# facebookresearch/spdl

Measured on AMD Instinct MI355X. Metric: images/sec device-resident JPEG→RGB224, 1/2/4/8×MI355X; % HBM roofline, higher is better.
Workload: dtype u8; 1 GPU; configs[1]: synthetic 480x640 q90 4:2:0 baseline JPEG resident in HBM -> RGB 224x224 u8 (scale bicubic decrease + centred pad, rgb24); global_batch=256, per_gpu_batch=256, distinct_images=32, lanes=4, hw_queues=4, entropy_threads=256, entropy_piece_bytes=131072

## Files before the change

spdl_amd/csrc/hj_common.h:

```cpp
#pragma once
#include <stddef.h>
#include <stdint.h>

#ifndef HJ_HD
#define HJ_HD __host__ __device__
#endif

namespace hj {

constexpr int kMaxComp = 4;

enum { kColorGray = 0, kColorYcbcr, kColorRgb, kColorCmyk, kColorYcck, kColorYcbcrk };
inline HJ_HD bool frame_color(int ncomp, const int32_t* h, const int32_t* v, const int* ids,
                              int adobe, int32_t* color) {
  bool all11 = true;
  for (int c = 0; c < ncomp; c++) all11 = all11 && h[c] == 1 && v[c] == 1;
  if (ncomp == 1) {
    *color = kColorGray;
  } else if (ncomp == 3) {
    const bool rgb = adobe == 0 || (ids[0] == 'R' && ids[1] == 'G' && ids[2] == 'B');
    if (rgb && !all11) return false;
    *color = rgb ? kColorRgb : kColorYcbcr;
  } else {
    if (!all11) return false;
// ... 69 lines not shown
  int32_t sub_lo;
  int32_t maxcode[18];
  int32_t valoff[17];
  uint8_t vals[256];
};

enum { kSwsX = 0, kSwsOne = 1, kSwsTwo = 2 };
enum SwsTable { kHlPos = 0, kHlCoef, kHcPos, kHcCoef, kVlPos, kVlCoef, kVcPos, kVcCoef, kVmode, kSwsTables };
struct SwsDesc {
  int32_t sw, sh;
  int32_t chr_w;
  int32_t full, gray;
  int32_t hl_taps, hc_taps, vl_taps, vc_taps;
  int32_t hl_size, hc_size, vl_size, vc_size;
  int32_t off[kSwsTables];
  int32_t rb;
  int32_t col_chunk;
  int32_t gbr;
  int32_t pre, pre_rl, pre_rc;
  int32_t yuv, hsub, vsub, chr_h;
};

struct ImageDesc {
  int64_t in_off;
  int64_t in_size;
  int64_t coef_off;
  int64_t plane_off[kMaxComp];
  int64_t seg_off;
  int64_t out_off;
  int64_t wt_off;
  int32_t seg_cap;
  int32_t width, height, ncomp;
  int32_t h_samp[kMaxComp], v_samp[kMaxComp];
  int32_t nblocks;
  int32_t plane_stride[kMaxComp];
  int32_t dx, dy, ow, oh;
  SwsDesc sws;
  int64_t ds_off;
  int32_t ds_cap;
  int32_t color;
  int64_t rec_off;
  int64_t rec_cap;
  int32_t pieces;
  int32_t chain_off;
  int32_t ds_wg0, idct_wg0;
  int32_t hs_wg0, hs_wgs;
  int32_t sws_wg0, sws_bands, sws_chunks;
  int64_t hbuf_off;
  int32_t refuse;
  int32_t pad_;
};

#ifndef HJ_SWS_LDS_KB
#define HJ_SWS_LDS_KB 32
#endif
constexpr int kSwsLdsBudget = HJ_SWS_LDS_KB * 1024;
constexpr int kSwsMaxCols = 256;
inline HJ_HD int sws_col_stride(int rows) { return 2 * (((rows + 5) >> 1) | 1); }

struct ImageInfo {
  int32_t status;
  int32_t width, height, ncomp, hmax, vmax, mcux, mcuy, bpm, nblocks, ri;
  int32_t scan_start;
  int32_t comp_h[kMaxComp], comp_v[kMaxComp];
  int32_t comp_bw[kMaxComp], comp_bh[kMaxComp];
  int32_t comp_w[kMaxComp], comp_hpx[kMaxComp];
  int32_t mcu_comp[kMaxBpm], mcu_dx[kMaxBpm], mcu_dy[kMaxBpm];
  int32_t dc_tab[kMaxComp], ac_tab[kMaxComp];
  uint16_t qt[kMaxComp][64];
  int32_t nseg;
  int32_t clean_len;
  int32_t sync_rounds;
  int32_t scan_end;
  int32_t ent_wide;
  int32_t multiscan;
  int32_t progressive;
  int32_t color;
  int32_t tab_off[8], tab_n[8];
  uint32_t tab_hash[8];
  int32_t lut_ref[8];
  int64_t tphase[4];
  int64_t dbg[4];
  int32_t sdiag[48];
};

constexpr int kDsChunk = 4096;
#ifndef HJ_IDCT_THREADS
#define HJ_IDCT_THREADS 256
#endif
constexpr int kIdctThreads = HJ_IDCT_THREADS;
constexpr int kHsRows = 16;
struct DsChunk {
  int32_t keep, rst, term;
  int32_t keep_pre, rst_pre;
  int32_t pad_[3];
};

struct SwsCsc {
  int32_t crv, cbu, cgu, cgv;
  int32_t y_coeff, y_offset, v2r, v2g, u2g, u2b;
};

#ifndef HJ_ABLATIONS
#define HJ_ABLATIONS 0
#endif
enum Ablate : int32_t {
  kAblSwsHpass = 0x100,
  kAblSwsVpass = 0x200,
  kAblSwsStore = 0x400,
  kAblIdctNone = 0x800,
  kAblEntWrite = 0x1000,
  kAblEntSync = 0x2000,
  kAblEntList = 0x4000,
  kAblEntDc = 0x8000,
  kAblEntDesc = 0x80000,
  kAblEntropy = kAblEntWrite | kAblEntSync | kAblEntList | kAblEntDc | kAblEntDesc,
  kAblNoMultiscan = 0x10000,
  kAblNoIdct = 0x20000,
  kAblNoOutput = 0x40000,
};

struct BatchParams {
  int32_t n;
  int32_t pix_fmt, dtype, idct;
  int32_t resize, filter;
  int32_t out_w, out_h;
  int32_t sub_bits;
  int32_t debug_mask;
  int32_t xcd_order;
  float mean[3], std[3];
  SwsCsc csc;
};
static_assert(sizeof(BatchParams) == 108 && offsetof(BatchParams, csc) == 68, "BatchParams layout");

struct EntropyParams {
  int32_t sub_bits;
  int32_t warm_slots;
  int32_t min_run_slots;
  int32_t chain_after;
  int32_t prio;
  int32_t ablate;
  int64_t handoff_ticks;
};

enum Status {
  kOk = 0,
  kErrNotJpeg = 1,
  kErrUnsupported = 2,
  kErrBadHeader = 3,
  kErrBadHuffman = 4,
  kErrTruncated = 5,
  kErrBadRestart = 6,
  kErrBadGeometry = 7,
  kErrDevice = 9,
  kErrHandoff = 11,
};

}
```

spdl_amd/csrc/hj_kernels.hip:

```cpp
#include <hip/hip_fp16.h>
#include <hip/hip_runtime.h>

#include "hj_common.h"
#include "hj_destuff.h"
#include "hj_idct.h"
#include "hj_launch.h"
#include "hj_sws_tile.h"

namespace hj {

__device__ __forceinline__ uint32_t rfl(uint32_t v) { return __builtin_amdgcn_readfirstlane(v); }


struct ParseScratch {
  ImageInfo info;
  uint16_t qt[4][64];
  uint8_t bits[8][17];
  uint8_t vals[8][256];
  int32_t have[8];
  int32_t qhave[4];
  int32_t maxcode[8][18];
  int32_t valoff[8][17];
  int32_t dqt_off[4], dqt_pq[4];
  int32_t dht_off[8], dht_n[8];
// ... 104 lines not shown
        if (in.comp_h[c] < 1 || in.comp_h[c] > 4 || in.comp_v[c] < 1 || in.comp_v[c] > 4 ||
            comp_tq[c] > 3)
          return kErrBadHeader;
      }
      if (!frame_color(nf, in.comp_h, in.comp_v, comp_id, adobe, &in.color)) return kErrUnsupported;
      have_sof = 1;
    } else if (m == 0xC3 || (m >= 0xC5 && m <= 0xC7) || (m >= 0xC9 && m <= 0xCB) ||
               (m >= 0xCD && m <= 0xCF)) {
      return kErrUnsupported;
    } else if (m == 0xEE) {
      if (n >= 12 && p[0] == 'A' && p[1] == 'd' && p[2] == 'o' && p[3] == 'b' && p[4] == 'e')
        adobe = p[11];
    } else if (m == 0xDD) {
      if (n < 2) return kErrBadHeader;
      in.ri = be16(p);
    } else if (m == 0xDA) {
      if (!have_sof) return kErrBadHeader;
      int ns = p[0];
      if (ns < 1 || ns > in.ncomp) return kErrBadHeader;
      in.multiscan = prog || ns != in.ncomp;
      in.progressive = prog;
      if (n < 1 + 2 * ns + 3) return kErrBadHeader;
      int32_t* order = s.order;
      for (int i = 0; i < kMaxComp; i++) order[i] = 0;
      for (int i = 0; i < ns; i++) {
        int cs = p[1 + 2 * i], c = -1;
        for (int k = 0; k < in.ncomp; k++)
          if (comp_id[k] == cs) c = k;
        if (c < 0) return kErrBadHeader;
        order[i] = c;
        in.dc_tab[c] = p[2 + 2 * i] >> 4;
        in.ac_tab[c] = p[2 + 2 * i] & 15;
        if (in.dc_tab[c] > 3 || in.ac_tab[c] > 3) return kErrBadHeader;
      }
      int ss = p[1 + 2 * ns], se = p[2 + 2 * ns], ahal = p[3 + 2 * ns];
      if (!in.multiscan && (ss != 0 || se != 63 || ahal != 0)) return kErrUnsupported;
      in.scan_start = pos;
      if (in.multiscan)
        for (int i = 0; i < in.ncomp; i++) order[i] = i;
      int hmax = 1, vmax = 1;
      for (int c = 0; c < in.ncomp; c++) {
        hmax = max(hmax, in.comp_h[c]);
        vmax = max(vmax, in.comp_v[c]);
      }
      in.hmax = hmax;
      in.vmax = vmax;
      for (int c = 0; c < in.ncomp; c++) {
        if (hmax % in.comp_h[c] || vmax % in.comp_v[c]) return kErrUnsupported;
        if (!s.qhave[comp_tq[c]] ||
            (!in.multiscan && (!s.have[in.dc_tab[c]] || !s.have[4 + in.ac_tab[c]])))
          return kErrBadHeader;
        in.comp_w[c] = (in.width * in.comp_h[c] + hmax - 1) / hmax;
        in.comp_hpx[c] = (in.height * in.comp_v[c] + vmax - 1) / vmax;
        s.qtsel[c] = comp_tq[c];
      }
      if (in.ncomp == 1) {
        in.comp_bw[0] = (in.comp_w[0] + 7) / 8;
        in.comp_bh[0] = (in.comp_hpx[0] + 7) / 8;
        in.mcux = in.comp_bw[0];
        in.mcuy = in.comp_bh[0];
        in.bpm = 1;
        in.mcu_comp[0] = 0;
        in.mcu_dx[0] = in.mcu_dy[0] = 0;
      } else {
        in.mcux = (in.width + 8 * hmax - 1) / (8 * hmax);
        in.mcuy = (in.height + 8 * vmax - 1) / (8 * vmax);
        int b = 0;
        for (int i = 0; i < (in.multiscan ? in.ncomp : ns); i++) {
          int c = order[i];
          in.comp_bw[c] = in.mcux * in.comp_h[c];
          in.comp_bh[c] = in.mcuy * in.comp_v[c];
          for (int y = 0; y < in.comp_v[c]; y++)
            for (int x = 0; x < in.comp_h[c]; x++) {
              if (b >= kMaxBpm) return kErrUnsupported;
              in.mcu_comp[b] = c;
              in.mcu_dx[b] = x;
              in.mcu_dy[b] = y;
              b++;
            }
        }
        in.bpm = b;
      }
      in.nblocks = in.mcux * in.mcuy * in.bpm;
      return kOk;
    }
  }
}

__global__ void __launch_bounds__(256, 8) parse_kernel(const uint8_t* __restrict__ bytes,
                                                    const ImageDesc* __restrict__ host_desc,
                                                    ImageDesc* __restrict__ desc,
                                                    ImageInfo* __restrict__ infos,
                                                    HuffTable* __restrict__ luts,
                                                    const uint4* __restrict__ host_tables,
                                                    uint4* __restrict__ tables, int64_t ntab16,
                                                    const uint32_t* __restrict__ host_work,
                                                    uint32_t* __restrict__ work, int nwork,
                                                    uint64_t* __restrict__ chain,
                                                    uint32_t* __restrict__ ds_map,
                                                    uint32_t* __restrict__ idct_map,
                                                    uint32_t* __restrict__ hs_map,
                                                    uint32_t* __restrict__ sws_map) {
  __shared__ ParseScratch s;
  __shared__ int st;
  __shared__ __attribute__((aligned(16))) uint8_t hdr[kHdrBytes];
  const int img = blockIdx.x, tid = threadIdx.x;
#if HJ_PARSE_PROF
  int64_t pt[8];
  int npt = 0;
  pt[npt++] = wall_clock64();
#define HJ_PT() (pt[npt++] = wall_clock64())
#else
#define HJ_PT() ((void)0)
#endif
  __shared__ __attribute__((aligned(16))) ImageDesc sdd;
  {
    static_assert(sizeof(ImageDesc) % 8 == 0, "descriptor copied in 8-byte words");
    const uint64_t* src = reinterpret_cast<const uint64_t*>((host_desc ? host_desc : desc) + img);
    uint64_t* dst = reinterpret_cast<uint64_t*>(desc + img);
    uint64_t* sdst = reinterpret_cast<uint64_t*>(&sdd);
    for (int i = tid; i < (int)(sizeof(ImageDesc) / 8); i += blockDim.x) {
      const uint64_t v = src[i];
      if (host_desc) dst[i] = v;
      sdst[i] = v;
    }
  }
  if (host_desc) {
    for (int64_t i = (int64_t)img * blockDim.x + tid; i < ntab16;
         i += (int64_t)gridDim.x * blockDim.x)
      tables[i] = host_tables[i];
    for (int i = img * blockDim.x + tid; i < nwork; i += gridDim.x * blockDim.x)
      work[i] = host_work[i];
  }
  __syncthreads();
  const ImageDesc& dd = sdd;
  for (int i = tid; i < dd.ds_cap; i += blockDim.x) ds_map[dd.ds_wg0 + i] = (uint32_t)img;
  for (int i = tid; i < (dd.nblocks + kIdctThreads - 1) / kIdctThreads; i += blockDim.x)
    idct_map[dd.idct_wg0 + i] = (uint32_t)img;
  for (int i = tid; i < dd.hs_wgs; i += blockDim.x) hs_map[dd.hs_wg0 + i] = (uint32_t)img;
  for (int i = tid; i < dd.sws_bands * dd.sws_chunks; i += blockDim.x)
    sws_map[dd.sws_wg0 + i] = (uint32_t)img;
  if (img == 0 && tid == 0) chain[0] = 0ull;
  if (dd.pieces > 1)
    for (int i = tid; i < dd.pieces * kChainGranules; i += blockDim.x)
      chain[kChainHead + dd.chain_off + i] = 0ull;
  {
    int* z = reinterpret_cast<int*>(&s);
    for (int i = tid; i < (int)(sizeof(ParseScratch) / 4); i += blockDim.x) z[i] = 0;
  }
  const int nh = (int)min(dd.in_size, (int64_t)kHdrBytes) & ~15;
  for (int i = tid; i < nh / 16; i += blockDim.x)
    reinterpret_cast<uint4*>(hdr)[i] = reinterpret_cast<const uint4*>(bytes + dd.in_off)[i];
  __syncthreads();
  HJ_PT();
  if (tid == 0) {
    const Bytes file{bytes + dd.in_off, (lds_u8*)hdr, nh};
    int rc = parse_headers(file, (int)dd.in_size, s);
    if (rc == kOk) {
      if (s.info.width != dd.width || s.info.height != dd.height || s.info.ncomp != dd.ncomp ||
          s.info.nblocks != dd.nblocks || s.info.color != dd.color)
        rc = kErrBadHeader;
      for (int c = 0; c < s.info.ncomp && rc == kOk; c++)
        if (s.info.comp_h[c] != dd.h_samp[c] || s.info.comp_v[c] != dd.v_samp[c])
          rc = kErrBadHeader;
      if (rc == kOk && s.info.ri > 0 &&
          (s.info.mcux * s.info.mcuy + s.info.ri - 1) / s.info.ri > dd.seg_cap)
// ... 3446 lines not shown
      {
        const int2 rn = wr ? ms_decode_refine<MsWBits>(S, si, soft, geo, in, d, cl, sizeu, lv,
                                                       masks, lane)
                           : ms_decode_refine<MsBits>(S, si, soft, geo, in, d, cl, sizeu, lv,
                                                      masks, lane);
        rc = ms_i(rn.x);
        nsym = ms_i(rn.y);
      }
#endif
#undef HJ_MS_SCAN
      ms_publish(S, si, 1 << 30);
      if (ms_lane0() && si < 16) {
        S.sdiag[3 * si] = (int32_t)(ts - tdec);
        S.sdiag[3 * si + 1] = (int32_t)(wall_clock64() - tdec);
        S.sdiag[3 * si + 2] = nsym;
#ifdef HJ_MS_PROF
        if (prof[1]) {
          S.sdiag[3 * si] = (int32_t)(prof[0] >> 8);
          S.sdiag[3 * si + 1] = (int32_t)(prof[1] >> 8);
          S.sdiag[3 * si + 2] = (int32_t)(prof[2] >> 8);
        }
#endif
      }
      if (ms_lane0()) {
        if (rc != kOk) atomicCAS(&S.err, kOk, rc);
        const int sss = ms_i(sc.ss), sah = ms_i(sc.ah);
        const int kind = !progu ? 3 : (sss == 0 ? 0 : (sah == 0 ? 1 : 2));
        atomicAdd(reinterpret_cast<unsigned long long*>(&S.tkind[kind]),
                  (unsigned long long)(wall_clock64() - ts));
        __hip_atomic_fetch_or(&S.done, 1ull << si, __ATOMIC_RELEASE, __HIP_MEMORY_SCOPE_WORKGROUP);
      }
    }
    __builtin_amdgcn_s_setprio(0);
  }
  __syncthreads();
  tph[2] = wall_clock64() - tdec;
#pragma unroll
  for (int i = 0; i < 4; i++) tdbg[i] = S.tkind[i];
  tdbg[3] = (int64_t)__builtin_amdgcn_s_memtime() - cdec;
  tph[1] = 0;
  if (S.err != kOk) {
    if (tid == 0) in.status = S.err;
    return;
  }
  for (int j = tid; j < nblocks; j += nt) {
    const int c = in.mcu_comp[j % in.bpm];
    uint4 q[16];
    const uint4* src = reinterpret_cast<const uint4*>(lv + (size_t)j * 64);
#pragma unroll
    for (int i = 0; i < 16; i++) q[i] = src[i];
    int32_t l[64];
#pragma unroll
    for (int i = 0; i < 16; i++) {
      l[4 * i] = (int32_t)q[i].x;
      l[4 * i + 1] = (int32_t)q[i].y;
      l[4 * i + 2] = (int32_t)q[i].z;
      l[4 * i + 3] = (int32_t)q[i].w;
    }
    uint32_t* out = ents + ((size_t)dd.coef_off + j) * 64;
    uint32_t n = 0;
#pragma unroll
    for (int k = 1; k < 64; k++) {
      if (l[k] != 0) {
        out[n++] = ((uint32_t)l[k] << 16) | (uint32_t)k;
      }
    }
    const int32_t dc = (int32_t)(int16_t)(uint16_t)((uint32_t)kDcBias + (uint32_t)l[0] * in.qt[c][0]);
    bdesc[(size_t)dd.coef_off + j] = make_uint2((uint32_t)j * 64u, n | ((uint32_t)dc << 16));
  }
  __syncthreads();
  if (tid == 0) {
    tph[3] = wall_clock64() - t0 - tph[0] - tph[1] - tph[2];
    for (int i = 0; i < 4; i++) in.tphase[i] = tph[i];
    for (int i = 0; i < 4; i++) in.dbg[i] = tdbg[i];
    for (int i = 0; i < 48; i++) in.sdiag[i] = S.sdiag[i];
    in.sync_rounds = S.nscans;
  }
}


constexpr int kBlkWords = 32;

typedef int16_t __attribute__((may_alias)) hj_i16_alias;

template <int NT>
__device__ __forceinline__ uint32_t slot_byte(uint32_t s) {
  return (s >> 1) * (uint32_t)NT * 4u + ((s & 1u) << 1);
}

template <int NT>
__device__ __forceinline__ void load_dequant(uint32_t (&sq)[kMaxComp][64], const ImageInfo& in,
                                             int tid) {
  for (int k = tid; k < kMaxComp * 64; k += NT)
    sq[k >> 6][k & 63] = slot_byte<NT>(kSlotOrder[k & 63]) | ((uint32_t)in.qt[k >> 6][k & 63] << 16);
}

template <int NT>
__device__ __forceinline__ void list_block(const uint32_t* __restrict__ ents, const uint2 bd,
                                           const int64_t coef_off, const int nblocks,
                                           const uint32_t* sqc, uint32_t* b32) {
#pragma unroll
  for (int w = 0; w < kBlkWords; w++) b32[w * NT] = w == 0 ? (bd.y >> 16) : 0u;
  uint8_t* blk = reinterpret_cast<uint8_t*>(b32);
  uint8_t* dummy = reinterpret_cast<uint8_t*>(b32 + kBlkWords * NT);
  const uint32_t cap = (uint32_t)nblocks * 64u;
  const uint32_t lo = bd.x & 3u, start = bd.x & ~3u;
  uint32_t count = min(bd.y & 0xFFFFu, 63u);
  if (start > cap - 64u) count = 0;
  const uint32_t hi_e = lo + count;
  const uint4* e4 = reinterpret_cast<const uint4*>(ents + (size_t)coef_off * 64 + start);
  const uint32_t n4 = (hi_e + 3u) >> 2;
  for (uint32_t i = 0; i < n4; i += 4) {
    uint4 q[4];
#pragma unroll
    for (int u = 0; u < 4; u++) q[u] = e4[min(i + u, n4 - 1u)];
#pragma unroll
    for (int u = 0; u < 4; u++) {
      const uint32_t w[4] = {q[u].x, q[u].y, q[u].z, q[u].w};
#pragma unroll
      for (int h = 0; h < 4; h++) {
        const uint32_t k = 4u * (i + u) + h;
        const uint32_t qs = sqc[w[h] & 63u];
        uint8_t* dst = k >= lo && k < hi_e ? blk + (qs & 0xFFFFu) : dummy;
        *reinterpret_cast<hj_i16_alias*>(dst) = (int16_t)pk_mul_lo16(w[h] >> 16, qs >> 16);
      }
    }
  }
}

typedef short hj_s16x2 __attribute__((ext_vector_type(2)));
__device__ __forceinline__ int32_t dot2(uint32_t a, uint32_t w, int32_t c) {
  return __builtin_amdgcn_sdot2(__builtin_bit_cast(hj_s16x2, a), __builtin_bit_cast(hj_s16x2, w),
                                c, false);
}
constexpr uint32_t pk16(int lo, int hi) {
  return (uint32_t)(uint16_t)(int16_t)lo | ((uint32_t)(uint16_t)(int16_t)hi << 16);
}
__device__ __forceinline__ uint32_t pack_lo16(uint32_t lo, uint32_t hi) {
  return __builtin_amdgcn_perm(hi, lo, 0x05040100u);
}
__device__ __forceinline__ void sidct8(uint32_t e0, uint32_t e1, uint32_t o0, uint32_t o1,
                                       int32_t bias, int32_t (&a)[4], int32_t (&b)[4]) {
  a[0] = dot2(e1, pk16(kW4, kW6), dot2(e0, pk16(kW4, kW2), bias));
  a[1] = dot2(e1, pk16(-kW4, -kW2), dot2(e0, pk16(kW4, kW6), bias));
  a[2] = dot2(e1, pk16(-kW4, kW2), dot2(e0, pk16(kW4, -kW6), bias));
  a[3] = dot2(e1, pk16(kW4, -kW6), dot2(e0, pk16(kW4, -kW2), bias));
  b[0] = dot2(o1, pk16(kW5, kW7), dot2(o0, pk16(kW1, kW3), 0));
  b[1] = dot2(o1, pk16(-kW1, -kW5), dot2(o0, pk16(kW3, -kW7), 0));
  b[2] = dot2(o1, pk16(kW7, kW3), dot2(o0, pk16(kW5, -kW1), 0));
  b[3] = dot2(o1, pk16(kW3, -kW1), dot2(o0, pk16(kW7, -kW5), 0));
}
template <int NT>
__device__ __forceinline__ uint4 blk_row(const uint32_t* b32, int i) {
  return make_uint4(b32[(4 * i) * NT], b32[(4 * i + 1) * NT], b32[(4 * i + 2) * NT],
                    b32[(4 * i + 3) * NT]);
}
template <int NT>
__device__ __forceinline__ void simple_idct_slots(const uint32_t* b32, int32_t (&px)[64]) {
  uint32_t r[8][8];
#pragma unroll
  for (int i = 0; i < 8; i++) {
    const uint4 q = blk_row<NT>(b32, i);
    int32_t a[4], b[4];
    sidct8(q.x, q.y, q.z, q.w, 1 << 10, a, b);
    const bool dc_only = ((q.x >> 16) | q.y | q.z | q.w) == 0u;
    const uint32_t dc = q.x << 3;
    r[i][0] = dc_only ? dc : (uint32_t)((int32_t)((uint32_t)a[0] + (uint32_t)b[0]) >> 11);
    r[i][7] = dc_only ? dc : (uint32_t)((int32_t)((uint32_t)a[0] - (uint32_t)b[0]) >> 11);
    r[i][1] = dc_only ? dc : (uint32_t)((int32_t)((uint32_t)a[1] + (uint32_t)b[1]) >> 11);
    r[i][6] = dc_only ? dc : (uint32_t)((int32_t)((uint32_t)a[1] - (uint32_t)b[1]) >> 11);
    r[i][2] = dc_only ? dc : (uint32_t)((int32_t)((uint32_t)a[2] + (uint32_t)b[2]) >> 11);
    r[i][5] = dc_only ? dc : (uint32_t)((int32_t)((uint32_t)a[2] - (uint32_t)b[2]) >> 11);
    r[i][3] = dc_only ? dc : (uint32_t)((int32_t)((uint32_t)a[3] + (uint32_t)b[3]) >> 11);
    r[i][4] = dc_only ? dc : (uint32_t)((int32_t)((uint32_t)a[3] - (uint32_t)b[3]) >> 11);
  }
#pragma unroll
  for (int k = 0; k < 8; k++) {
    int32_t a[4], b[4];
    sidct8(pack_lo16(r[0][k], r[2][k]), pack_lo16(r[4][k], r[6][k]), pack_lo16(r[1][k], r[3][k]),
           pack_lo16(r[5][k], r[7][k]), kW4 * ((1 << 19) / kW4), a, b);
    px[k] = clip_u8_opaque((int32_t)((uint32_t)a[0] + (uint32_t)b[0]) >> 20);
    px[8 + k] = clip_u8_opaque((int32_t)((uint32_t)a[1] + (uint32_t)b[1]) >> 20);
    px[16 + k] = clip_u8_opaque((int32_t)((uint32_t)a[2] + (uint32_t)b[2]) >> 20);
    px[24 + k] = clip_u8_opaque((int32_t)((uint32_t)a[3] + (uint32_t)b[3]) >> 20);
    px[32 + k] = clip_u8_opaque((int32_t)((uint32_t)a[3] - (uint32_t)b[3]) >> 20);
    px[40 + k] = clip_u8_opaque((int32_t)((uint32_t)a[2] - (uint32_t)b[2]) >> 20);
    px[48 + k] = clip_u8_opaque((int32_t)((uint32_t)a[1] - (uint32_t)b[1]) >> 20);
    px[56 + k] = clip_u8_opaque((int32_t)((uint32_t)a[0] - (uint32_t)b[0]) >> 20);
  }
}

template <int NT, int IDCT>
__device__ __forceinline__ void idct_block(const uint32_t* b32, int32_t (&px)[64]) {
  if (IDCT == 0) {
    simple_idct_slots<NT>(b32, px);
    return;
  }
  int32_t blk[64];
#pragma unroll
  for (int i = 0; i < 8; i++) {
    const uint4 q = blk_row<NT>(b32, i);
    blk[8 * i + 0] = sext16(q.x);
    blk[8 * i + 2] = sext16(q.x >> 16);
    blk[8 * i + 4] = sext16(q.y);
    blk[8 * i + 6] = sext16(q.y >> 16);
    blk[8 * i + 1] = sext16(q.z);
    blk[8 * i + 3] = sext16(q.z >> 16);
    blk[8 * i + 5] = sext16(q.w);
    blk[8 * i + 7] = sext16(q.w >> 16);
  }
  if (IDCT == 2) {
#pragma unroll
    for (int i = 0; i < 64; i++) px[i] = blk[i] & 255;
  } else {
    islow_block(blk, px);
  }
}

__device__ __forceinline__ void xcd_order(uint32_t& bx, uint32_t& by, uint32_t& bz) {
  const uint32_t n_wg = gridDim.x * gridDim.y * gridDim.z, full = n_wg & ~7u;
  uint32_t lin = bx + gridDim.x * (by + gridDim.y * bz);
  if (lin < full) lin = (lin & 7u) * (full >> 3) + (lin >> 3);
  bx = lin % gridDim.x;
  by = (lin / gridDim.x) % gridDim.y;
  bz = lin / (gridDim.x * gridDim.y);
}

template <int IDCT>
__global__ void __launch_bounds__(kIdctThreads) idct_kernel(const uint32_t* __restrict__ ents,
                                                            const uint2* __restrict__ bdesc,
                                                            const ImageDesc* __restrict__ desc,
                                                            const ImageInfo* __restrict__ infos,
                                                            uint8_t* __restrict__ planes,
                                                            const uint32_t* __restrict__ idct_map,
                                                            const int xcd) {
  __shared__ __attribute__((aligned(16))) uint32_t sblk[kBlkWords + 1][kIdctThreads];
  __shared__ uint32_t sq[kMaxComp][64];
  uint32_t gx = blockIdx.x, gy = blockIdx.y, gz = blockIdx.z;
  if (xcd) xcd_order(gx, gy, gz);
  const bool flat = idct_map != nullptr;
  const int img = flat ? (int)idct_map[gx] : (int)gy;
  const int tile = flat ? (int)gx - desc[img].idct_wg0 : (int)gx;
  const int j = tile * kIdctThreads + threadIdx.x;
  const ImageInfo& in = infos[img];
  if (in.status != kOk || tile * kIdctThreads >= in.nblocks) return;
  load_dequant<kIdctThreads>(sq, in, threadIdx.x);
  __syncthreads();
  if (j >= in.nblocks) return;
  const ImageDesc& dd = desc[img];
  const int bpm = in.bpm;
  const int mcu = j / bpm, b = j - mcu * bpm;
  const int c = in.mcu_comp[b];
  const int mx = mcu % in.mcux, my = mcu / in.mcux;
  int bx, by;
  if (in.ncomp == 1) {
    bx = mx;
    by = my;
  } else {
    bx = mx * in.comp_h[c] + in.mcu_dx[b];
    by = my * in.comp_v[c] + in.mcu_dy[b];
  }
  uint32_t* b32 = &sblk[0][threadIdx.x];
  list_block<kIdctThreads>(ents, bdesc[(size_t)dd.coef_off + j], dd.coef_off, in.nblocks, sq[c],
                           b32);
  int32_t px[64];
  idct_block<kIdctThreads, IDCT>(b32, px);
  const int stride = dd.plane_stride[c];
  uint8_t* dst = planes + dd.plane_off[c] + (size_t)by * 8 * stride + bx * 8;
#pragma unroll
  for (int r = 0; r < 8; r++) {
    uint2 v;
    v.x = (uint32_t)px[8 * r] | ((uint32_t)px[8 * r + 1] << 8) | ((uint32_t)px[8 * r + 2] << 16) |
          ((uint32_t)px[8 * r + 3] << 24);
    v.y = (uint32_t)px[8 * r + 4] | ((uint32_t)px[8 * r + 5] << 8) |
          ((uint32_t)px[8 * r + 6] << 16) | ((uint32_t)px[8 * r + 7] << 24);
    *reinterpret_cast<uint2*>(dst + (size_t)r * stride) = v;
  }
}


constexpr int32_t kFix1402 = 91881, kFix1772 = 116130, kFix0714 = 46802, kFix0344 = 22553;

__device__ __forceinline__ void ycc_rgb(int y, int cb, int cr, int* rgb) {
  const int32_t x_cb = cb - 128, x_cr = cr - 128;
  const int32_t cr_r = (kFix1402 * x_cr + 32768) >> 16;
  const int32_t cb_b = (kFix1772 * x_cb + 32768) >> 16;
  const int32_t g = ((-kFix0344 * x_cb + 32768) + (-kFix0714 * x_cr)) >> 16;
  rgb[0] = clip_u8(y + cr_r);
  rgb[1] = clip_u8(y + g);
  rgb[2] = clip_u8(y + cb_b);
}

__device__ __forceinline__ uint16_t to_f16_bits(float f, int dtype) {
  if (dtype == 1) return __half_as_ushort(__float2half_rn(f));
  uint32_t x = __float_as_uint(f);
  if ((x & 0x7FFFFFFFu) > 0x7F800000u) return (uint16_t)((x >> 16) | 0x40u);
  x += 0x7FFFu + ((x >> 16) & 1u);
  return (uint16_t)(x >> 16);
}

__device__ __forceinline__ void store_rgb(void* out, int64_t base, int fmt, int dtype, int ow,
                                          int oh, int x, int y, const int* rgb,
                                          const BatchParams& p) {
  const bool planar = fmt == 0 || fmt == 1;
  const bool swap = fmt == 1 || fmt == 3;
  const int64_t pl = (int64_t)ow * oh;
#pragma unroll
  for (int ch = 0; ch < 3; ch++) {
    const int v = rgb[swap ? 2 - ch : ch];
    const int64_t oi = base + (planar ? ch * pl + (int64_t)y * ow + x : ((int64_t)y * ow + x) * 3 + ch);
    if (dtype == 0) {
      static_cast<uint8_t*>(out)[oi] = (uint8_t)v;
    } else {
      float f = __fdiv_rn((float)v, 255.0f);
      f = __fsub_rn(f, p.mean[ch]);
      f = __fdiv_rn(f, p.std[ch]);
      static_cast<uint16_t*>(out)[oi] = to_f16_bits(f, dtype);
    }
  }
}

__global__ void __launch_bounds__(256) csc_kernel(const uint8_t* __restrict__ planes,
                                                  const ImageDesc* __restrict__ desc,
                                                  const ImageInfo* __restrict__ infos,
                                                  void* __restrict__ out, const BatchParams p,
                                                  int32_t* __restrict__ host_status) {
  const int img = blockIdx.y;
  const ImageInfo& in = infos[img];
  if (host_status && blockIdx.x == 0 && threadIdx.x == 0) host_status[img] = in.status;
  if (in.status != kOk) return;
  const ImageDesc& dd = desc[img];
  const int W = in.width, H = in.height;
  const int64_t npx = (int64_t)W * H;
  for (int64_t i = (int64_t)blockIdx.x * blockDim.x + threadIdx.x; i < npx;
       i += (int64_t)gridDim.x * blockDim.x) {
    const int y = (int)(i / W), x = (int)(i - (int64_t)y * W);
    const int lx = x * in.comp_h[0] / in.hmax, ly = y * in.comp_v[0] / in.vmax;
    const int yv = planes[dd.plane_off[0] + (int64_t)ly * dd.plane_stride[0] + lx];
    int rgb[3];
    if (in.ncomp == 1) {
      rgb[0] = rgb[1] = rgb[2] = yv;
    } else {
      const int cx1 = x * in.comp_h[1] / in.hmax, cy1 = y * in.comp_v[1] / in.vmax;
      const int cx2 = x * in.comp_h[2] / in.hmax, cy2 = y * in.comp_v[2] / in.vmax;
      const int cb = planes[dd.plane_off[1] + (int64_t)cy1 * dd.plane_stride[1] + cx1];
      const int cr = planes[dd.plane_off[2] + (int64_t)cy2 * dd.plane_stride[2] + cx2];
      if (in.color == kColorRgb) {
        rgb[0] = yv;
        rgb[1] = cb;
        rgb[2] = cr;
      } else {
        ycc_rgb(yv, cb, cr, rgb);
      }
    }
    store_rgb(out, dd.out_off, p.pix_fmt, p.dtype, W, H, x, y, rgb, p);
  }
}


typedef short hj_short2 __attribute__((ext_vector_type(2)));
// ... 808 lines not shown
        o[3 * i + 1] = (uint8_t)c1[i];
        o[3 * i + 2] = (uint8_t)c2[i];
      }
    }
  } else {
#pragma unroll
    for (int c = 0; c < 3; c++) {
      const uint32_t* cv = c == 0 ? c0 : c == 1 ? c1 : c2;
      uint8_t* o = base + c * pl + (int64_t)y * w + x0;
      if (npx == PX && ((uintptr_t)o & (4u * SW - 1u)) == 0u) {
        uint32_t wv[SW];
#pragma unroll
        for (int k = 0; k < SW; k++)
          wv[k] = cv[4 * k] | cv[4 * k + 1] << 8 | cv[4 * k + 2] << 16 | cv[4 * k + 3] << 24;
        rgbu_store<SW>(o, wv);
      } else {
        for (int i = 0; i < npx; i++) o[i] = (uint8_t)cv[i];
      }
    }
  }
}

__global__ void __launch_bounds__(256) rgb_unscaled_kernel(const uint8_t* __restrict__ planes,
                                                           const ImageDesc* __restrict__ desc,
                                                           const ImageInfo* __restrict__ infos,
                                                           uint8_t* __restrict__ out,
                                                           const BatchParams p,
                                                           int32_t* __restrict__ host_status) {
  constexpr int PX = kRgbPx, YW = PX / 4, CW = PX / 8;
  const int img = blockIdx.y;
  const ImageInfo& in = infos[img];
  if (host_status && blockIdx.x == 0 && threadIdx.x == 0) host_status[img] = in.status;
  if (in.status != kOk) return;
  const ImageDesc& dd = desc[img];
  const int w = dd.ow, h = dd.oh;
  const uint32_t ngr = (uint32_t)(w + PX - 1) / PX;
  const uint32_t total = ngr * (uint32_t)h;
  const int vsub = in.comp_v[0] > in.comp_v[1] ? 1 : 0;
  const bool planar = p.pix_fmt == 0 || p.pix_fmt == 1;
  const bool swap = p.pix_fmt == 1 || p.pix_fmt == 3;
  const int64_t pl = (int64_t)w * h;
  const uint8_t* y_pl = planes + dd.plane_off[0];
  const uint8_t* u_pl = planes + dd.plane_off[1];
  const uint8_t* v_pl = planes + dd.plane_off[2];
  uint8_t* base = out + dd.out_off;
  for (uint32_t g = blockIdx.x * blockDim.x + threadIdx.x; g < total; g += gridDim.x * blockDim.x) {
    const int y = (int)(g / ngr), x0 = (int)(g - (uint32_t)y * ngr) * PX;
    const int npx = x0 + PX <= w ? PX : w - x0;
    uint32_t yw[YW], uw[CW], vw[CW];
    rgbu_load<YW>(y_pl + (int64_t)y * dd.plane_stride[0] + x0, yw);
    rgbu_load<CW>(u_pl + (int64_t)(y >> vsub) * dd.plane_stride[1] + (x0 >> 1), uw);
    rgbu_load<CW>(v_pl + (int64_t)(y >> vsub) * dd.plane_stride[2] + (x0 >> 1), vw);
    rgbu_group<PX>(yw, uw, vw, base, pl, w, y, x0, npx, p, planar, swap);
  }
}

template <int IDCT>
__global__ void __launch_bounds__(kFusedThreads) idct_rgb_kernel(const uint32_t* __restrict__ ents,
                                                       const uint2* __restrict__ bdesc,
                                                       const ImageDesc* __restrict__ desc,
                                                       const ImageInfo* __restrict__ infos,
                                                       uint8_t* __restrict__ out,
                                                       const BatchParams p,
                                                       int32_t* __restrict__ host_status) {
  __shared__ __attribute__((aligned(16))) uint32_t sblk[kBlkWords + 1][kFusedThreads];
  __shared__ uint32_t sq[kMaxComp][64];
  const int img = blockIdx.y, tid = threadIdx.x;
  const ImageInfo& in = infos[img];
  if (host_status && blockIdx.x == 0 && tid == 0) host_status[img] = in.status;
  if (in.status != kOk) return;
  const ImageDesc& dd = desc[img];
  const int bpm = in.bpm;
  const int tw = kFusedThreads / bpm;
  const int tiles_x = (in.mcux + tw - 1) / tw;
  if ((int)blockIdx.x >= tiles_x * in.mcuy) return;
  const int my = (int)blockIdx.x / tiles_x, mx0 = ((int)blockIdx.x - my * tiles_x) * tw;
  const int nm = min(tw, in.mcux - mx0);
  const int hy = 8 * in.comp_v[0];
  const int ys = tw * 16, cs = tw * 8;
  const bool act = tid < nm * bpm;
  const int m = tid / bpm, b = tid - m * bpm;
  load_dequant<kFusedThreads>(sq, in, tid);
  __syncthreads();
  int32_t px[64];
  if (act) {
    const int j = (my * in.mcux + mx0 + m) * bpm + b;
    list_block<kFusedThreads>(ents, bdesc[(size_t)dd.coef_off + j], dd.coef_off, in.nblocks,
                              sq[in.mcu_comp[b]], &sblk[0][tid]);
    idct_block<kFusedThreads, IDCT>(&sblk[0][tid], px);
  }
  __syncthreads();
  uint8_t* tl = reinterpret_cast<uint8_t*>(&sblk[0][0]);
  uint8_t* tu = tl + hy * ys;
  uint8_t* tv = tu + 8 * cs;
  if (act) {
    const int c = in.mcu_comp[b];
    uint8_t* dst = c == 0 ? tl + in.mcu_dy[b] * 8 * ys + m * 16 + in.mcu_dx[b] * 8
                          : (c == 1 ? tu : tv) + m * 8;
    const int st = c == 0 ? ys : cs;
#pragma unroll
    for (int r = 0; r < 8; r++) {
      uint2 v;
      v.x = (uint32_t)px[8 * r] | ((uint32_t)px[8 * r + 1] << 8) | ((uint32_t)px[8 * r + 2] << 16) |
            ((uint32_t)px[8 * r + 3] << 24);
      v.y = (uint32_t)px[8 * r + 4] | ((uint32_t)px[8 * r + 5] << 8) |
            ((uint32_t)px[8 * r + 6] << 16) | ((uint32_t)px[8 * r + 7] << 24);
      *reinterpret_cast<uint2*>(dst + r * st) = v;
    }
  }
  __syncthreads();
  const int w = dd.ow, h = dd.oh;
  const int x_base = mx0 * 16, y_base = my * hy;
  const int cols = min(nm * 16, w - x_base), rows = min(hy, h - y_base);
  const int ngr = (cols + 7) >> 3;
  const int vsub = hy == 16 ? 1 : 0;
  const bool planar = p.pix_fmt == 0 || p.pix_fmt == 1;
  const bool swap = p.pix_fmt == 1 || p.pix_fmt == 3;
  const int64_t pl = (int64_t)w * h;
  uint8_t* base = out + dd.out_off;
  for (int g = tid; g < ngr * rows; g += kFusedThreads) {
    const int r = g / ngr, xl = (g - r * ngr) * 8;
    const uint2 yq = *reinterpret_cast<const uint2*>(tl + r * ys + xl);
    const uint32_t yw[2] = {yq.x, yq.y};
    const uint32_t uw[1] = {*reinterpret_cast<const uint32_t*>(tu + (r >> vsub) * cs + (xl >> 1))};
    const uint32_t vw[1] = {*reinterpret_cast<const uint32_t*>(tv + (r >> vsub) * cs + (xl >> 1))};
    rgbu_group<8>(yw, uw, vw, base, pl, w, y_base + r, x_base + xl, min(8, cols - xl), p, planar,
                  swap);
  }
}

__global__ void __launch_bounds__(256) cmyk_kernel(const ImageDesc* __restrict__ desc,
                                                   const ImageInfo* __restrict__ infos,
                                                   uint8_t* __restrict__ planes) {
  const int img = blockIdx.y;
  const ImageInfo& in = infos[img];
  if (in.status != kOk || (in.color != kColorCmyk && in.color != kColorYcck)) return;
  const ImageDesc& dd = desc[img];
  const int wq = (in.width + 3) >> 2, stride = dd.plane_stride[0];
  const bool ycck = in.color == kColorYcck;
  const int64_t nq = (int64_t)wq * in.height;
  for (int64_t i = (int64_t)blockIdx.x * blockDim.x + threadIdx.x; i < nq;
       i += (int64_t)gridDim.x * blockDim.x) {
    const int y = (int)(i / wq), x = 4 * (int)(i - (int64_t)y * wq);
    const int64_t o = (int64_t)y * stride + x;
    uint32_t* p0 = reinterpret_cast<uint32_t*>(planes + dd.plane_off[0] + o);
    uint32_t* p1 = reinterpret_cast<uint32_t*>(planes + dd.plane_off[1] + o);
    uint32_t* p2 = reinterpret_cast<uint32_t*>(planes + dd.plane_off[2] + o);
    const uint32_t k4 = *reinterpret_cast<const uint32_t*>(planes + dd.plane_off[3] + o);
    const uint32_t a = *p0, b = *p1, c = *p2;
    uint32_t ra = 0, rb = 0, rc = 0;
#pragma unroll
    for (int j = 0; j < 4; j++) {
      const int k = (int)((k4 >> (8 * j)) & 255u);
      const int va = (int)((a >> (8 * j)) & 255u), vb = (int)((b >> (8 * j)) & 255u),
                vc = (int)((c >> (8 * j)) & 255u);
      int oa, ob, oc;
      if (ycck) {
        oa = ((255 - va) * k * 257) >> 16;
        ob = ((((128 - vb) * k) * 257) >> 16) + 128;
        oc = ((((128 - vc) * k) * 257) >> 16) + 128;
      } else {
        oa = (va * k * 257) >> 16;
        ob = (vb * k * 257) >> 16;
        oc = (vc * k * 257) >> 16;
      }
      ra |= (uint32_t)(oa & 255) << (8 * j);
      rb |= (uint32_t)(ob & 255) << (8 * j);
      rc |= (uint32_t)(oc & 255) << (8 * j);
    }
    *p0 = ra;
    *p1 = rb;
    *p2 = rc;
  }
}

__constant__ float kYuv2Rgb[10][3][3] = {
    {{1.1644f, 0.0000f, 1.8337f}, {1.1644f, -0.2181f, -0.5451f}, {1.1644f, 2.1606f, 0.0000f}},
    {{1.1644f, 0.0000f, 1.8337f}, {1.1644f, -0.2181f, -0.5451f}, {1.1644f, 2.1606f, 0.0000f}},
    {{1.1644f, 0.0000f, 1.8337f}, {1.1644f, -0.2181f, -0.5451f}, {1.1644f, 2.1606f, 0.0000f}},
    {{1.1644f, 0.0000f, 1.6301f}, {1.1644f, -0.3864f, -0.8289f}, {1.1644f, 2.0726f, 0.0000f}},
    {{1.1644f, 0.0000f, 1.6325f}, {1.1644f, -0.4007f, -0.8315f}, {1.1644f, 2.0633f, 0.0000f}},
    {{1.1644f, 0.0000f, 1.6325f}, {1.1644f, -0.4007f, -0.8315f}, {1.1644f, 2.0633f, 0.0000f}},
    {{1.1644f, 0.0000f, 1.8351f}, {1.1644f, -0.2639f, -0.5550f}, {1.1644f, 2.1262f, 0.0000f}},
    {{1.1644f, 0.0000f, 1.8337f}, {1.1644f, -0.2181f, -0.5451f}, {1.1644f, 2.1606f, 0.0000f}},
    {{1.1689f, 0.0000f, 1.7237f}, {1.1689f, -0.1924f, -0.6679f}, {1.1689f, 2.1992f, 0.0000f}},
    {{1.1689f, 0.0000f, 1.7237f}, {1.1689f, -0.1924f, -0.6679f}, {1.1689f, 2.1992f, 0.0000f}},
};

__device__ __forceinline__ uint8_t clamp8f(float x) {
  return x < 0.0f ? 0 : (x > 255.0f ? 255 : (uint8_t)x);
}
// ... 146 lines not shown
```

Measured before the change: 594,900 images/sec.

## Micro-optimize IDCT path: magic-number divmod, SDWA scatter, packed clip, DC-bias folding

Replaces integer div/mod in IDCT block indexing with precomputed magic-multiply divmod stored in ImageInfo. Rewrites the coefficient scatter into LDS with SDWA inline asm and batched quant-table gathers. It also folds the DC-only shortcut into the row-pass bias and uses scalar-operand dot2 seeds. Column outputs are packed with v_ashr_pk_u8_i32 so rows come out as uint2 directly. The aim is fewer ALU instructions in the IDCT stage, at the cost of gfx-specific inline asm and new ImageInfo fields.

```diff
diff --git a/spdl_amd/csrc/hj_common.h b/spdl_amd/csrc/hj_common.h
--- a/spdl_amd/csrc/hj_common.h
+++ b/spdl_amd/csrc/hj_common.h
@@ -175,7 +175,39 @@
   int64_t tphase[4];
   int64_t dbg[4];
   int32_t sdiag[48];
-};
+  uint32_t bpm_magic, mcux_magic;
+};
+
+#ifndef HJ_IDCT_INDEX
+#define HJ_IDCT_INDEX 1
+#endif
+inline HJ_HD uint32_t idct_div_magic(uint32_t d) { return 0xFFFFFFFFu / d; }
+struct IdctDivMod {
+  uint32_t q, r;
+};
+inline HJ_HD IdctDivMod idct_divmod(uint32_t n, uint32_t d, uint32_t magic) {
+#if HJ_IDCT_INDEX
+  uint32_t q = (uint32_t)(((uint64_t)n * magic) >> 32);
+  uint32_t r = n - q * d;
+  if (r >= d) {
+    q += 1;
+    r -= d;
+  }
+  return {q, r};
+#else
+  return {n / d, n % d};
+#endif
+}
+struct IdctBlockPos {
+  int c, bx, by;
+};
+inline HJ_HD IdctBlockPos idct_block_pos(const ImageInfo& in, uint32_t j) {
+  const IdctDivMod m = idct_divmod(j, (uint32_t)in.bpm, in.bpm_magic);
+  const IdctDivMod p = idct_divmod(m.q, (uint32_t)in.mcux, in.mcux_magic);
+  const int b = (int)m.r, c = in.mcu_comp[b];
+  if (in.ncomp == 1) return {c, (int)p.r, (int)p.q};
+  return {c, (int)p.r * in.comp_h[c] + in.mcu_dx[b], (int)p.q * in.comp_v[c] + in.mcu_dy[b]};
+}
 
 constexpr int kDsChunk = 4096;
 #ifndef HJ_IDCT_THREADS
diff --git a/spdl_amd/csrc/hj_kernels.hip b/spdl_amd/csrc/hj_kernels.hip
--- a/spdl_amd/csrc/hj_kernels.hip
+++ b/spdl_amd/csrc/hj_kernels.hip
@@ -210,6 +210,8 @@
         in.bpm = b;
       }
       in.nblocks = in.mcux * in.mcuy * in.bpm;
+      in.bpm_magic = idct_div_magic((uint32_t)in.bpm);
+      in.mcux_magic = idct_div_magic((uint32_t)in.mcux);
       return kOk;
     }
   }
@@ -3822,6 +3824,24 @@
 constexpr int kBlkWords = 32;
 
 typedef int16_t __attribute__((may_alias)) hj_i16_alias;
+typedef __attribute__((address_space(3))) hj_i16_alias hj_lds_i16;
+typedef __attribute__((address_space(3))) uint32_t hj_lds_u32;
+
+#ifndef HJ_IDCT_SEED
+#define HJ_IDCT_SEED 1
+#endif
+#ifndef HJ_IDCT_DCBIAS
+#define HJ_IDCT_DCBIAS 1
+#endif
+#ifndef HJ_IDCT_PACK
+#define HJ_IDCT_PACK 1
+#endif
+#ifndef HJ_IDCT_SCATTER
+#define HJ_IDCT_SCATTER 1
+#endif
+#ifndef HJ_IDCT_GATHER
+#define HJ_IDCT_GATHER 1
+#endif
 
 template <int NT>
 __device__ __forceinline__ uint32_t slot_byte(uint32_t s) {
@@ -3841,8 +3861,13 @@
                                            const uint32_t* sqc, uint32_t* b32) {
 #pragma unroll
   for (int w = 0; w < kBlkWords; w++) b32[w * NT] = w == 0 ? (bd.y >> 16) : 0u;
+#if HJ_IDCT_SCATTER
+  const uint32_t blk_a = (uint32_t)(uintptr_t)(hj_lds_u32*)b32;
+  const uint32_t dummy_a = blk_a + (uint32_t)(kBlkWords * NT * 4);
+#else
   uint8_t* blk = reinterpret_cast<uint8_t*>(b32);
   uint8_t* dummy = reinterpret_cast<uint8_t*>(b32 + kBlkWords * NT);
+#endif
   const uint32_t cap = (uint32_t)nblocks * 64u;
   const uint32_t lo = bd.x & 3u, start = bd.x & ~3u;
   uint32_t count = min(bd.y & 0xFFFFu, 63u);
@@ -3854,15 +3879,43 @@
     uint4 q[4];
 #pragma unroll
     for (int u = 0; u < 4; u++) q[u] = e4[min(i + u, n4 - 1u)];
+#if HJ_IDCT_GATHER
+    uint32_t qsv[16];
+#pragma unroll
+    for (int u = 0; u < 4; u++) {
+      qsv[4 * u] = sqc[q[u].x & 63u];
+      qsv[4 * u + 1] = sqc[q[u].y & 63u];
+      qsv[4 * u + 2] = sqc[q[u].z & 63u];
+      qsv[4 * u + 3] = sqc[q[u].w & 63u];
+    }
+#endif
 #pragma unroll
     for (int u = 0; u < 4; u++) {
       const uint32_t w[4] = {q[u].x, q[u].y, q[u].z, q[u].w};
 #pragma unroll
       for (int h = 0; h < 4; h++) {
         const uint32_t k = 4u * (i + u) + h;
+#if HJ_IDCT_GATHER
+        const uint32_t qs = qsv[4 * u + h];
+#else
         const uint32_t qs = sqc[w[h] & 63u];
+#endif
+#if HJ_IDCT_SCATTER
+        uint32_t in_a, prod;
+        asm("v_add_u32_sdwa %0, %1, %2 dst_sel:DWORD dst_unused:UNUSED_PAD src0_sel:DWORD "
+            "src1_sel:WORD_0"
+            : "=v"(in_a)
+            : "v"(blk_a), "v"(qs));
+        asm("v_mul_lo_u16_sdwa %0, %1, %2 dst_sel:DWORD dst_unused:UNUSED_PAD src0_sel:WORD_1 "
+            "src1_sel:WORD_1"
+            : "=v"(prod)
+            : "v"(w[h]), "v"(qs));
+        const uint32_t a32 = k - lo < count ? in_a : dummy_a;
+        *reinterpret_cast<hj_lds_i16*>(a32) = (int16_t)prod;
+#else
         uint8_t* dst = k >= lo && k < hi_e ? blk + (qs & 0xFFFFu) : dummy;
         *reinterpret_cast<hj_i16_alias*>(dst) = (int16_t)pk_mul_lo16(w[h] >> 16, qs >> 16);
+#endif
       }
     }
   }
@@ -3879,16 +3932,34 @@
 __device__ __forceinline__ uint32_t pack_lo16(uint32_t lo, uint32_t hi) {
   return __builtin_amdgcn_perm(hi, lo, 0x05040100u);
 }
+__device__ __forceinline__ int32_t dot2_seed(uint32_t a, uint32_t w, int32_t c) {
+#if HJ_IDCT_SEED
+  int32_t d;
+  asm("v_dot2_i32_i16 %0, %1, %2, %3" : "=v"(d) : "v"(a), "s"(w), "v"(c));
+  return d;
+#else
+  return dot2(a, w, c);
+#endif
+}
+__device__ __forceinline__ int32_t dot2_seed0(uint32_t a, uint32_t w) {
+#if HJ_IDCT_SEED
+  int32_t d;
+  asm("v_dot2_i32_i16 %0, %1, %2, 0" : "=v"(d) : "v"(a), "s"(w));
+  return d;
+#else
+  return dot2(a, w, 0);
+#endif
+}
 __device__ __forceinline__ void sidct8(uint32_t e0, uint32_t e1, uint32_t o0, uint32_t o1,
                                        int32_t bias, int32_t (&a)[4], int32_t (&b)[4]) {
-  a[0] = dot2(e1, pk16(kW4, kW6), dot2(e0, pk16(kW4, kW2), bias));
-  a[1] = dot2(e1, pk16(-kW4, -kW2), dot2(e0, pk16(kW4, kW6), bias));
-  a[2] = dot2(e1, pk16(-kW4, kW2), dot2(e0, pk16(kW4, -kW6), bias));
-  a[3] = dot2(e1, pk16(kW4, -kW6), dot2(e0, pk16(kW4, -kW2), bias));
-  b[0] = dot2(o1, pk16(kW5, kW7), dot2(o0, pk16(kW1, kW3), 0));
-  b[1] = dot2(o1, pk16(-kW1, -kW5), dot2(o0, pk16(kW3, -kW7), 0));
-  b[2] = dot2(o1, pk16(kW7, kW3), dot2(o0, pk16(kW5, -kW1), 0));
-  b[3] = dot2(o1, pk16(kW3, -kW1), dot2(o0, pk16(kW7, -kW5), 0));
+  a[0] = dot2(e1, pk16(kW4, kW6), dot2_seed(e0, pk16(kW4, kW2), bias));
+  a[1] = dot2(e1, pk16(-kW4, -kW2), dot2_seed(e0, pk16(kW4, kW6), bias));
+  a[2] = dot2(e1, pk16(-kW4, kW2), dot2_seed(e0, pk16(kW4, -kW6), bias));
+  a[3] = dot2(e1, pk16(kW4, -kW6), dot2_seed(e0, pk16(kW4, -kW2), bias));
+  b[0] = dot2(o1, pk16(kW5, kW7), dot2_seed0(o0, pk16(kW1, kW3)));
+  b[1] = dot2(o1, pk16(-kW1, -kW5), dot2_seed0(o0, pk16(kW3, -kW7)));
+  b[2] = dot2(o1, pk16(kW7, kW3), dot2_seed0(o0, pk16(kW5, -kW1)));
+  b[3] = dot2(o1, pk16(kW3, -kW1), dot2_seed0(o0, pk16(kW7, -kW5)));
 }
 template <int NT>
 __device__ __forceinline__ uint4 blk_row(const uint32_t* b32, int i) {
@@ -3896,37 +3967,73 @@
                     b32[(4 * i + 3) * NT]);
 }
 template <int NT>
-__device__ __forceinline__ void simple_idct_slots(const uint32_t* b32, int32_t (&px)[64]) {
-  uint32_t r[8][8];
+__device__ __forceinline__ void simple_idct_rows(const uint32_t* b32, uint32_t (&r)[8][8]) {
 #pragma unroll
   for (int i = 0; i < 8; i++) {
     const uint4 q = blk_row<NT>(b32, i);
     int32_t a[4], b[4];
+    const bool dc_only = ((q.x >> 16) | q.y | q.z | q.w) == 0u;
+#if HJ_IDCT_DCBIAS
+    sidct8(q.x, q.y, q.z, q.w, (1 << 10) + (dc_only ? sext16(q.x) : 0), a, b);
+#pragma unroll
+    for (int k = 0; k < 4; k++) {
+      r[i][k] = (uint32_t)((int32_t)((uint32_t)a[k] + (uint32_t)b[k]) >> 11);
+      r[i][7 - k] = (uint32_t)((int32_t)((uint32_t)a[k] - (uint32_t)b[k]) >> 11);
+    }
+#else
     sidct8(q.x, q.y, q.z, q.w, 1 << 10, a, b);
-    const bool dc_only = ((q.x >> 16) | q.y | q.z | q.w) == 0u;
     const uint32_t dc = q.x << 3;
-    r[i][0] = dc_only ? dc : (uint32_t)((int32_t)((uint32_t)a[0] + (uint32_t)b[0]) >> 11);
-    r[i][7] = dc_only ? dc : (uint32_t)((int32_t)((uint32_t)a[0] - (uint32_t)b[0]) >> 11);
-    r[i][1] = dc_only ? dc : (uint32_t)((int32_t)((uint32_t)a[1] + (uint32_t)b[1]) >> 11);
-    r[i][6] = dc_only ? dc : (uint32_t)((int32_t)((uint32_t)a[1] - (uint32_t)b[1]) >> 11);
-    r[i][2] = dc_only ? dc : (uint32_t)((int32_t)((uint32_t)a[2] + (uint32_t)b[2]) >> 11);
-    r[i][5] = dc_only ? dc : (uint32_t)((int32_t)((uint32_t)a[2] - (uint32_t)b[2]) >> 11);
-    r[i][3] = dc_only ? dc : (uint32_t)((int32_t)((uint32_t)a[3] + (uint32_t)b[3]) >> 11);
-    r[i][4] = dc_only ? dc : (uint32_t)((int32_t)((uint32_t)a[3] - (uint32_t)b[3]) >> 11);
-  }
+#pragma unroll
+    for (int k = 0; k < 4; k++) {
+      r[i][k] = dc_only ? dc : (uint32_t)((int32_t)((uint32_t)a[k] + (uint32_t)b[k]) >> 11);
+      r[i][7 - k] = dc_only ? dc : (uint32_t)((int32_t)((uint32_t)a[k] - (uint32_t)b[k]) >> 11);
+    }
+#endif
+  }
+}
+__device__ __forceinline__ void simple_idct_col(const uint32_t (&r)[8][8], int k,
+                                                int32_t (&s)[8]) {
+  int32_t a[4], b[4];
+  sidct8(pack_lo16(r[0][k], r[2][k]), pack_lo16(r[4][k], r[6][k]), pack_lo16(r[1][k], r[3][k]),
+         pack_lo16(r[5][k], r[7][k]), kW4 * ((1 << 19) / kW4), a, b);
+#pragma unroll
+  for (int u = 0; u < 4; u++) {
+    s[u] = (int32_t)((uint32_t)a[u] + (uint32_t)b[u]);
+    s[7 - u] = (int32_t)((uint32_t)a[u] - (uint32_t)b[u]);
+  }
+}
+template <int NT>
+__device__ __forceinline__ void simple_idct_slots(const uint32_t* b32, int32_t (&px)[64]) {
+  uint32_t r[8][8];
+  simple_idct_rows<NT>(b32, r);
 #pragma unroll
   for (int k = 0; k < 8; k++) {
-    int32_t a[4], b[4];
-    sidct8(pack_lo16(r[0][k], r[2][k]), pack_lo16(r[4][k], r[6][k]), pack_lo16(r[1][k], r[3][k]),
-           pack_lo16(r[5][k], r[7][k]), kW4 * ((1 << 19) / kW4), a, b);
-    px[k] = clip_u8_opaque((int32_t)((uint32_t)a[0] + (uint32_t)b[0]) >> 20);
-    px[8 + k] = clip_u8_opaque((int32_t)((uint32_t)a[1] + (uint32_t)b[1]) >> 20);
-    px[16 + k] = clip_u8_opaque((int32_t)((uint32_t)a[2] + (uint32_t)b[2]) >> 20);
-    px[24 + k] = clip_u8_opaque((int32_t)((uint32_t)a[3] + (uint32_t)b[3]) >> 20);
-    px[32 + k] = clip_u8_opaque((int32_t)((uint32_t)a[3] - (uint32_t)b[3]) >> 20);
-    px[40 + k] = clip_u8_opaque((int32_t)((uint32_t)a[2] - (uint32_t)b[2]) >> 20);
-    px[48 + k] = clip_u8_opaque((int32_t)((uint32_t)a[1] - (uint32_t)b[1]) >> 20);
-    px[56 + k] = clip_u8_opaque((int32_t)((uint32_t)a[0] - (uint32_t)b[0]) >> 20);
+    int32_t s[8];
+    simple_idct_col(r, k, s);
+#pragma unroll
+    for (int j = 0; j < 8; j++) px[8 * j + k] = clip_u8_opaque(s[j] >> 20);
+  }
+}
+
+__device__ __forceinline__ uint32_t clip_pair(int32_t a, int32_t b) {
+  uint32_t u;
+  asm("v_ashr_pk_u8_i32 %0, %1, %2, 20" : "=v"(u) : "v"(a), "v"(b));
+  return u;
+}
+__device__ __forceinline__ uint32_t clip_pack4(int32_t a, int32_t b, int32_t c, int32_t d) {
+  return __builtin_amdgcn_perm(clip_pair(c, d), clip_pair(a, b), 0x05040100u);
+}
+template <int NT>
+__device__ __forceinline__ void simple_idct_packed(const uint32_t* b32, uint2 (&rows)[8]) {
+  uint32_t r[8][8];
+  simple_idct_rows<NT>(b32, r);
+  int32_t s[8][8];
+#pragma unroll
+  for (int k = 0; k < 8; k++) simple_idct_col(r, k, s[k]);
+#pragma unroll
+  for (int j = 0; j < 8; j++) {
+    rows[j].x = clip_pack4(s[0][j], s[1][j], s[2][j], s[3][j]);
+    rows[j].y = clip_pack4(s[4][j], s[5][j], s[6][j], s[7][j]);
   }
 }
 
@@ -3954,6 +4061,25 @@
     for (int i = 0; i < 64; i++) px[i] = blk[i] & 255;
   } else {
     islow_block(blk, px);
+  }
+}
+
+template <int NT, int IDCT>
+__device__ __forceinline__ void idct_block_rows(const uint32_t* b32, uint2 (&rows)[8]) {
+#if HJ_IDCT_PACK
+  if (IDCT == 0) {
+    simple_idct_packed<NT>(b32, rows);
+    return;
+  }
+#endif
+  int32_t px[64];
+  idct_block<NT, IDCT>(b32, px);
+#pragma unroll
+  for (int r = 0; r < 8; r++) {
+    rows[r].x = (uint32_t)px[8 * r] | ((uint32_t)px[8 * r + 1] << 8) |
+                ((uint32_t)px[8 * r + 2] << 16) | ((uint32_t)px[8 * r + 3] << 24);
+    rows[r].y = (uint32_t)px[8 * r + 4] | ((uint32_t)px[8 * r + 5] << 8) |
+                ((uint32_t)px[8 * r + 6] << 16) | ((uint32_t)px[8 * r + 7] << 24);
   }
 }
 
@@ -3988,34 +4114,17 @@
   __syncthreads();
   if (j >= in.nblocks) return;
   const ImageDesc& dd = desc[img];
-  const int bpm = in.bpm;
-  const int mcu = j / bpm, b = j - mcu * bpm;
-  const int c = in.mcu_comp[b];
-  const int mx = mcu % in.mcux, my = mcu / in.mcux;
-  int bx, by;
-  if (in.ncomp == 1) {
-    bx = mx;
-    by = my;
-  } else {
-    bx = mx * in.comp_h[c] + in.mcu_dx[b];
-    by = my * in.comp_v[c] + in.mcu_dy[b];
-  }
+  const IdctBlockPos bp = idct_block_pos(in, (uint32_t)j);
+  const int c = bp.c;
   uint32_t* b32 = &sblk[0][threadIdx.x];
   list_block<kIdctThreads>(ents, bdesc[(size_t)dd.coef_off + j], dd.coef_off, in.nblocks, sq[c],
                            b32);
-  int32_t px[64];
-  idct_block<kIdctThreads, IDCT>(b32, px);
+  uint2 rows[8];
+  idct_block_rows<kIdctThreads, IDCT>(b32, rows);
   const int stride = dd.plane_stride[c];
-  uint8_t* dst = planes + dd.plane_off[c] + (size_t)by * 8 * stride + bx * 8;
-#pragma unroll
-  for (int r = 0; r < 8; r++) {
-    uint2 v;
-    v.x = (uint32_t)px[8 * r] | ((uint32_t)px[8 * r + 1] << 8) | ((uint32_t)px[8 * r + 2] << 16) |
-          ((uint32_t)px[8 * r + 3] << 24);
-    v.y = (uint32_t)px[8 * r + 4] | ((uint32_t)px[8 * r + 5] << 8) |
-          ((uint32_t)px[8 * r + 6] << 16) | ((uint32_t)px[8 * r + 7] << 24);
-    *reinterpret_cast<uint2*>(dst + (size_t)r * stride) = v;
-  }
+  uint8_t* dst = planes + dd.plane_off[c] + (size_t)bp.by * 8 * stride + bp.bx * 8;
+#pragma unroll
+  for (int r = 0; r < 8; r++) *reinterpret_cast<uint2*>(dst + (size_t)r * stride) = rows[r];
 }
 
 
@@ -4990,12 +5099,12 @@
   const int m = tid / bpm, b = tid - m * bpm;
   load_dequant<kFusedThreads>(sq, in, tid);
   __syncthreads();
-  int32_t px[64];
+  uint2 px[8];
   if (act) {
     const int j = (my * in.mcux + mx0 + m) * bpm + b;
     list_block<kFusedThreads>(ents, bdesc[(size_t)dd.coef_off + j], dd.coef_off, in.nblocks,
                               sq[in.mcu_comp[b]], &sblk[0][tid]);
-    idct_block<kFusedThreads, IDCT>(&sblk[0][tid], px);
+    idct_block_rows<kFusedThreads, IDCT>(&sblk[0][tid], px);
   }
   __syncthreads();
   uint8_t* tl = reinterpret_cast<uint8_t*>(&sblk[0][0]);
@@ -5007,14 +5116,7 @@
                           : (c == 1 ? tu : tv) + m * 8;
     const int st = c == 0 ? ys : cs;
 #pragma unroll
-    for (int r = 0; r < 8; r++) {
-      uint2 v;
-      v.x = (uint32_t)px[8 * r] | ((uint32_t)px[8 * r + 1] << 8) | ((uint32_t)px[8 * r + 2] << 16) |
-            ((uint32_t)px[8 * r + 3] << 24);
-      v.y = (uint32_t)px[8 * r + 4] | ((uint32_t)px[8 * r + 5] << 8) |
-            ((uint32_t)px[8 * r + 6] << 16) | ((uint32_t)px[8 * r + 7] << 24);
-      *reinterpret_cast<uint2*>(dst + r * st) = v;
-    }
+    for (int r = 0; r < 8; r++) *reinterpret_cast<uint2*>(dst + r * st) = px[r];
   }
   __syncthreads();
   const int w = dd.ow, h = dd.oh;
```

New measurement: 608,900 images/sec, median of 6. 2.4% higher.
